# CX9898/BSMR-SDDMM

Measured on AMD Instinct MI355X. Metric: SDDMM GFLOP/s, higher is better.
Workload: dtype f16

## Files before the change

bsmr-sddmm_amd/csrc/gemm_format.hpp:

```cpp
#pragma once

#include <algorithm>
#include <cstdint>
#include <vector>

#include "bsmr_hip.h"
#include "tile_format.hpp"

namespace bsmr {

constexpr uint32_t kGemmWavesM = 2, kGemmWavesN = 4, kGemmWaves = kGemmWavesM * kGemmWavesN;
__host__ __device__ constexpr uint32_t gemmSlabSlot(uint32_t tp, uint32_t r, uint32_t c) { return tp * 256u + (r & 3u) * 64u + (r >> 2) * 16u + c; }
constexpr uint32_t kGemmPassTiles = 16;
constexpr uint32_t kGemmNoEntry = 0xFFFFFFFFu;
constexpr uint32_t kGemmMaxOffset = 8191u;
constexpr uint32_t kGemmSlabStrips = 8;
constexpr uint32_t kGemmWordSlack = 1024;

struct GemmItem {
    uint32_t group;
    uint32_t firstBlock;
    uint32_t listBase;
    uint32_t pad;
};

__host__ __device__ inline void gemmItemPlace(uint32_t i, uint32_t G, uint32_t S, uint32_t& group, uint32_t& strip) {
    const uint32_t slabs = (S + kGemmSlabStrips - 1u) / kGemmSlabStrips;
    uint32_t slab = i / (kGemmSlabStrips * G);
    if (slab >= slabs) slab = slabs - 1u;
    const uint32_t width = slab + 1u < slabs ? kGemmSlabStrips : S - kGemmSlabStrips * (slabs - 1u);
    const uint32_t rem = i - slab * kGemmSlabStrips * G;
    group = rem / width;
    strip = slab * kGemmSlabStrips + rem % width;
}

struct GemmFormatHost {
    uint32_t PM = 0, NB = 0, numGroups = 0, numStrips = 0, passes = 0;
    bool fullGrid = false;
    std::vector<uint32_t> panelRows;
    std::vector<uint32_t> colOf;
    std::vector<GemmItem> items;
    std::vector<uint32_t> rowStart;
    std::vector<uint32_t> lists;
    std::vector<uint32_t> words;
    uint64_t numTiles = 0;
    uint32_t maxListWords = 0;
    size_t bytes() const {
        return 4 * (panelRows.size() + colOf.size() + rowStart.size() + lists.size() + words.size()) + sizeof(GemmItem) * items.size();
    }
};

inline bool gemmShapeOk(uint32_t PM, uint32_t NB) {
    return (PM == 8 || PM == 16) && (NB == 8 || NB == 12 || NB == 16 || NB == 20);
}

inline int packGemm(const HostDense& hd, uint32_t PM, uint32_t NB, GemmFormatHost& out, bool balanceColumns = true) {
    if (!gemmShapeOk(PM, NB)) return BSMR_ERR_INVALID_ARG;
    const uint32_t P = hd.numPanels, TM = PM * 16;
    const uint32_t G = (P + PM - 1) / PM, NCB = (hd.N + 15) / 16, S = (NCB + NB - 1) / NB;
    const uint32_t m = PM / kGemmWavesM, n = NB / kGemmWavesN, Q = (m * n + kGemmPassTiles - 1) / kGemmPassTiles, L = kGemmWaves * Q;
    out = GemmFormatHost();
    out.PM = PM; out.NB = NB; out.numGroups = G; out.numStrips = S; out.passes = Q;
    if (P == 0 || NCB == 0 || hd.entries() == 0) return BSMR_OK;
    if ((uint64_t)G * S > 0x3FFFFFFFull || hd.entries() > 0xFFFFFFF0ull) return BSMR_ERR_INVALID_ARG;
    if ((uint64_t)hd.nnz * 4u > 0xFFFFFFFCull) return BSMR_ERR_INVALID_ARG;
    out.panelRows.assign((size_t)G * TM, hd.panelRows.empty() ? 0u : hd.panelRows[0]);
    std::vector<uint32_t> rowPos((size_t)P * 16);
    if (balanceColumns) {
        std::vector<uint32_t> weight((size_t)P * 16, 0), order((size_t)P * 16);
        for (uint32_t p = 0; p < P; ++p)
            for (uint64_t e = hd.offsets[p]; e < hd.offsets[p + 1]; ++e) ++weight[(size_t)p * 16 + hd.row[e]];
        for (uint32_t i = 0; i < P * 16; ++i) order[i] = i;
        std::stable_sort(order.begin(), order.end(), [&](uint32_t a, uint32_t b) { return weight[a] > weight[b]; });
        const uint32_t bins = 2 * G, half = TM / 2;
        for (uint32_t rank = 0; rank < P * 16; ++rank) {
            const uint32_t round = rank / bins, pos = rank % bins, bin = (round & 1u) ? bins - 1u - pos : pos;
            rowPos[order[rank]] = (bin / 2) * TM + (bin % 2) * half + round;
        }
    } else {
        for (uint32_t i = 0; i < P * 16; ++i) rowPos[i] = i;
    }
    for (uint32_t i = 0; i < P * 16; ++i) out.panelRows[rowPos[i]] = hd.panelRows[i];
    const uint32_t TN = NB * 16;
    std::vector<uint32_t> slotOf(hd.N);
    out.colOf.assign((size_t)S * TN, 0u);
    if (balanceColumns) {
        std::vector<uint32_t> degree(hd.N, 0), hot;
        for (uint64_t e = 0; e < hd.entries(); ++e) ++degree[hd.col[e]];
        uint64_t fullest = 0;
        for (uint32_t st = 0; st < S; ++st) {
            uint64_t sum = 0;
            for (uint32_t c = st * TN; c < std::min<uint64_t>(hd.N, (uint64_t)(st + 1) * TN); ++c) sum += degree[c];
            fullest = std::max(fullest, sum);
        }
        const bool lopsided = fullest * S > 2ull * hd.entries();
        const uint64_t threshold = lopsided ? 2ull * hd.entries() / std::max<uint32_t>(1u, hd.N) + 1ull : ~0ull;
        for (uint32_t c = 0; c < hd.N; ++c)
            if (degree[c] > threshold) hot.push_back(c);
        std::stable_sort(hot.begin(), hot.end(), [&](uint32_t a, uint32_t b) { return degree[a] > degree[b]; });
        std::vector<uint32_t> filled(S, 0);
        for (uint32_t rank = 0; rank < hot.size(); ++rank) {
            const uint32_t round = rank / S, pos = rank % S, strip = (round & 1u) ? S - 1u - pos : pos;
            slotOf[hot[rank]] = strip * TN + filled[strip]++;
        }
        uint32_t strip = 0;
        for (uint32_t c = 0; c < hd.N; ++c) {
            if (degree[c] > threshold) continue;
            while (filled[strip] == TN) ++strip;
            slotOf[c] = strip * TN + filled[strip]++;
        }
    } else {
        for (uint32_t c = 0; c < hd.N; ++c) slotOf[c] = c;
    }
    for (uint32_t c = 0; c < hd.N; ++c) out.colOf[slotOf[c]] = c;
    std::vector<uint32_t> itemOf((size_t)G * S, 0xFFFFFFFFu);
    std::vector<uint8_t> used((size_t)G * S, 0);
    for (uint32_t p = 0; p < P; ++p)
        for (uint64_t e = hd.offsets[p]; e < hd.offsets[p + 1]; ++e)
            used[(size_t)(rowPos[(size_t)p * 16 + hd.row[e]] / TM) * S + slotOf[hd.col[e]] / TN] = 1;
    for (uint32_t i = 0; i < G * S; ++i) {
        uint32_t g, st;
        gemmItemPlace(i, G, S, g, st);
        if (!used[(size_t)g * S + st]) continue;
        itemOf[(size_t)g * S + st] = (uint32_t)out.items.size();
        GemmItem it;
        it.group = g;
        it.firstBlock = st * NB;
        it.listBase = (uint32_t)(out.items.size() * (L + 1));
        it.pad = 0;
        out.items.push_back(it);
    }
    out.fullGrid = out.items.size() == (size_t)G * S;
    const size_t I = out.items.size();
    out.numTiles = (uint64_t)I * PM * NB;
    if (I * (size_t)(L + 1) > 0xFFFFFFFFull || I * (size_t)TM > 0xFFFFFFFFull) return BSMR_ERR_INVALID_ARG;
    out.lists.assign(I * (L + 1), 0);
    out.rowStart.assign(I * TM, 0xFFFFFFFFu);
    auto locate = [&](uint32_t p, uint64_t e, size_t& item, uint32_t& list, uint32_t& slot, uint32_t& rowInWave, uint32_t& rowInTile) {
        const uint32_t place = rowPos[(size_t)p * 16 + hd.row[e]];
        const uint32_t g = place / TM, pj = (place % TM) / 16u;
        const uint32_t slotCol = slotOf[hd.col[e]];
        const uint32_t cb = slotCol >> 4, s = cb / NB, bj = cb % NB;
        const uint32_t wm = pj / m, tm = pj % m, wn = bj / n, tn = bj % n;
        const uint32_t t = tm * n + tn, q = t / kGemmPassTiles, tp = t % kGemmPassTiles;
        const uint32_t r = place & 15u, c = slotCol & 15u;
        item = itemOf[(size_t)g * S + s];
        list = (wm * kGemmWavesN + wn) * Q + q;
        slot = gemmSlabSlot(tp, r, c);
        rowInWave = tm * 16 + r;
        rowInTile = pj * 16 + r;
    };
    for (uint32_t p = 0; p < P; ++p)
        for (uint64_t e = hd.offsets[p]; e < hd.offsets[p + 1]; ++e) {
            size_t item; uint32_t list, slot, rw, rt;
            locate(p, e, item, list, slot, rw, rt);
            ++out.lists[item * (L + 1) + list + 1];
            uint32_t& rs = out.rowStart[item * TM + rt];
            rs = std::min(rs, hd.idx[e]);
        }
    for (uint32_t& v : out.rowStart)
        if (v == 0xFFFFFFFFu) v = 0;
    uint64_t at = 0;
    for (size_t item = 0; item < I; ++item) {
        uint32_t* ls = &out.lists[item * (L + 1)];
        uint64_t run = at;
        for (uint32_t l = 0; l <= L; ++l) {
            const uint32_t cnt = ls[l];
            out.maxListWords = std::max(out.maxListWords, (cnt + 3u) & ~3u);
            run += (cnt + 3u) & ~3u;
            if (run > 0xFFFFFFF0ull) return BSMR_ERR_INVALID_ARG;
            ls[l] = (uint32_t)run;
        }
        at = run;
    }
    if (at > 0xFFFFFFF0ull) return BSMR_ERR_INVALID_ARG;
    out.words.assign((size_t)at + kGemmWordSlack, kGemmNoEntry);
    std::vector<uint32_t> fill(out.lists.size());
    for (size_t item = 0; item < I; ++item)
        for (uint32_t l = 0; l < L; ++l) fill[item * (L + 1) + l] = out.lists[item * (L + 1) + l];
    std::vector<uint64_t> keys(hd.entries());
    for (uint32_t p = 0; p < P; ++p)
        for (uint64_t e = hd.offsets[p]; e < hd.offsets[p + 1]; ++e) {
            size_t item; uint32_t list, slot, rw, rt;
            locate(p, e, item, list, slot, rw, rt);
            const uint32_t off = hd.idx[e] - out.rowStart[item * TM + rt];
            if (off >= kGemmMaxOffset) return BSMR_ERR_BAD_PLAN;
            const uint32_t word = slot | (rw << 12) | (off << 19);
            uint32_t& pos = fill[item * (L + 1) + list];
            keys[e] = ((uint64_t)rw << 45) | ((uint64_t)off << 32) | word;
            out.words[pos++] = (uint32_t)e;
        }
    std::vector<uint64_t> scratch;
    for (size_t item = 0; item < I; ++item)
        for (uint32_t l = 0; l < L; ++l) {
            const uint32_t b = out.lists[item * (L + 1) + l], e = fill[item * (L + 1) + l];
            scratch.resize(e - b);
            for (uint32_t i = b; i < e; ++i) scratch[i - b] = keys[out.words[i]];
            std::sort(scratch.begin(), scratch.end());
            for (uint32_t i = b; i < e; ++i) out.words[i] = (uint32_t)scratch[i - b];
        }
    return BSMR_OK;
}

}
```

bsmr-sddmm_amd/csrc/gemm_kernels.hpp:

```cpp
#pragma once

#include <hip/hip_runtime.h>
#include <stdint.h>

#include "gemm_format.hpp"
#include "sddmm_kernels.hpp"

namespace bsmr {

constexpr uint32_t kGemmBK = 64;
constexpr uint32_t kGemmRowBytes = kGemmBK * 2u;
__host__ __device__ constexpr uint32_t gemmSwz16(uint32_t row) { return (row >> 1) & 7u; }
__host__ __device__ constexpr uint32_t gemmSwz32(uint32_t row) { return ((row >> 1) & 1u) | (((row >> 3) & 1u) * 6u); }
constexpr uint32_t gemmStageBytes(int PM, int NB) { return (uint32_t)(PM + NB) * 16u * kGemmRowBytes; }
constexpr uint32_t kGemmSlabBytes = kGemmPassTiles * 1024u;
constexpr uint32_t gemmRingBytes(int PM, int NB) {
    return 2u * gemmStageBytes(PM, NB) > kGemmWaves * kGemmSlabBytes ? 2u * gemmStageBytes(PM, NB) : kGemmWaves * kGemmSlabBytes;
}
constexpr size_t gemmLdsBytes(int PM, int NB) { return gemmRingBytes(PM, NB) + (size_t)PM * 16u * 4u; }

#if defined(BSMR_GEMM_LAB)
#define GEMM_LAB_ARG , uint32_t labSkip, unsigned long long* labStamps
#define GEMM_LAB_SKIP(bit) (labSkip & (1u << (bit)))
#define GEMM_LAB_STAMPS unsigned long long labStamp[8] = {0, 0, 0, 0, 0, 0, 0, 0}
#define GEMM_LAB_STAMP(i) labStamp[i] = __builtin_amdgcn_s_memrealtime()
#define GEMM_LAB_STAMPS_OUT                                                                              \
    if (labStamps && lane == 0)                                                                          \
        for (uint32_t i = 0; i < 8u; ++i) labStamps[((size_t)blockIdx.x * kGemmWaves + wave) * 8u + i] = labStamp[i]
#else
#define GEMM_LAB_ARG
#define GEMM_LAB_SKIP(bit) false
#define GEMM_LAB_STAMPS
#define GEMM_LAB_STAMP(i)
#define GEMM_LAB_STAMPS_OUT
#endif

__device__ __forceinline__ void gemmKeep(const u32x4& x) {
#if defined(__HIP_DEVICE_COMPILE__)
    asm volatile("" ::"v"(x));
#else
    (void)x;
#endif
}

constexpr uint32_t kGemmDumpHigh = 64764u;
__device__ __forceinline__ void gemmDumpTile(const f32x4& a, uint32_t tileAddr, bool high) {
#if defined(__HIP_DEVICE_COMPILE__)
#pragma clang diagnostic push
#pragma clang diagnostic ignored "-Winline-asm"
    if (!high)
        asm volatile("s_mov_b32 m0, %4\n\ts_nop 0\n\tds_write_addtid_b32 %0\n\tds_write_addtid_b32 %1 offset:256\n\t"
                     "ds_write_addtid_b32 %2 offset:512\n\tds_write_addtid_b32 %3 offset:768"
                     ::"v"(a[0]), "v"(a[1]), "v"(a[2]), "v"(a[3]), "s"(tileAddr) : "memory", "m0");
    else
        asm volatile("s_mov_b32 m0, %4\n\ts_nop 0\n\tds_write_addtid_b32 %0 offset:64764\n\tds_write_addtid_b32 %1 offset:65020\n\t"
                     "ds_write_addtid_b32 %2 offset:65276\n\tds_write_addtid_b32 %3 offset:65532"
                     ::"v"(a[0]), "v"(a[1]), "v"(a[2]), "v"(a[3]), "s"(tileAddr - kGemmDumpHigh) : "memory", "m0");
#pragma clang diagnostic pop
#else
    (void)a; (void)tileAddr; (void)high;
#endif
}
__device__ __forceinline__ uint32_t gemmLdsAddress(const void* p) {
    return (uint32_t)(uintptr_t)(__attribute__((address_space(3))) const void*)p;
}

template <uint32_t DMAS>
__device__ __forceinline__ void gemmStagePart(const uint8_t* src, uint32_t srcBytes, uint8_t* dst, uint32_t wave, const uint32_t* voff, uint32_t kOff) {
    const auto rsrc = __builtin_amdgcn_make_buffer_rsrc(const_cast<uint8_t*>(src), 0, srcBytes, 0x00020000);
#pragma unroll
    for (uint32_t j = 0; j < DMAS; ++j)
        __builtin_amdgcn_raw_ptr_buffer_load_lds(rsrc, (__attribute__((address_space(3))) void*)(dst + (wave * DMAS + j) * 1024u), 16, voff[j], kOff, 0, 0);
}
#if !defined(BSMR_GEMM_BRANCHY_STORES)
__device__ __forceinline__ void gemmStoreEntry(float* P, bool live, uint32_t index, float val) {
    const auto rsrc = __builtin_amdgcn_make_buffer_rsrc(P, 0, 0xFFFFFFFC, 0x00020000);
    __builtin_amdgcn_raw_buffer_store_b32(__builtin_bit_cast(uint32_t, val), rsrc, live ? index << 2 : 0xFFFFFFFFu, 0, 0);
}
#endif
template <uint32_t ADMAS, uint32_t BDMAS>
__device__ __forceinline__ void gemmStage(const uint8_t* A, uint32_t aBytes, const uint8_t* B, uint32_t bBytes, uint8_t* stage, uint32_t bAt,
                                          uint32_t wave, const uint32_t* voffA, const uint32_t* voffB, uint32_t kOff) {
    gemmStagePart<BDMAS>(B, bBytes, stage + bAt, wave, voffB, kOff);
    gemmStagePart<ADMAS>(A, aBytes, stage, wave, voffA, kOff);
}
__device__ __forceinline__ uint32_t gemmRowOfLane(const uint32_t* __restrict__ rows8, uint32_t sub) {
    uint32_t id = rows8[0];
#pragma unroll
    for (uint32_t k = 1; k < 8; ++k) id = sub == k ? rows8[k] : id;
    return id;
}

template <int KT, int PM, int NB, int MODE, bool SRC32 = false>
__global__ void __launch_bounds__(kGemmWaves * kWave, 2)
denseGemm(const void* __restrict__ Aop, const void* __restrict__ Bop, uint32_t aBytes, uint32_t bBytes,
          const uint32_t* __restrict__ panelRows, const uint32_t* __restrict__ colOf, const GemmItem* __restrict__ items,
          const uint32_t* __restrict__ rowStart,
          const uint32_t* __restrict__ lists, const uint32_t* __restrict__ words, float* __restrict__ P, uint32_t N,
          uint32_t gridG, uint32_t gridS, uint32_t fullGrid, Batch batch GEMM_LAB_ARG) {
    constexpr uint32_t ESZ = SRC32 ? 4u : 2u, K = (kGemmRowBytes / ESZ) * KT, TM = PM * 16u, TN = NB * 16u;
    constexpr uint32_t KSUB = SRC32 ? 1u : 2u;
    constexpr uint32_t m = PM / kGemmWavesM, n = NB / kGemmWavesN, Q = (m * n + kGemmPassTiles - 1u) / kGemmPassTiles, L = kGemmWaves * Q;
    constexpr uint32_t ADMAS = PM / 4u, BDMAS = NB / 4u;
    static_assert(PM % 4 == 0 && NB % 4 == 0, "a stage is filled in whole 1-KiB pieces per wave");
    constexpr uint32_t stageBytes = gemmStageBytes(PM, NB), bAt = TM * kGemmRowBytes;
    constexpr uint32_t rowTableAt = gemmRingBytes(PM, NB);
    constexpr uint32_t kGemmWordChunk = m * n > 32u ? 4u : 8u;
    constexpr bool kPlainDump = m * n > 32u;

    extern __shared__ __attribute__((aligned(16))) uint8_t lds[];
    const uint32_t itemId = xcdContiguous(blockIdx.x, gridDim.x);
    uint32_t group, firstBlock, listBase;
    if (fullGrid) {
        gemmItemPlace(itemId, gridG, gridS, group, firstBlock);
        firstBlock *= (uint32_t)NB;
        listBase = itemId * (L + 1u);
    } else {
        const GemmItem item = items[itemId];
        group = item.group;
        firstBlock = item.firstBlock;
        listBase = item.listBase;
    }
    const uint32_t wave = __builtin_amdgcn_readfirstlane(threadIdx.x >> 6), lane = threadIdx.x & 63u;
    const uint32_t wm = wave / kGemmWavesN, wn = wave % kGemmWavesN;
    const uint32_t r = lane & 15u, g = lane >> 4;
    GEMM_LAB_STAMPS;
    GEMM_LAB_STAMP(0);

    const uint8_t* Ab = static_cast<const uint8_t*>(Aop) + (size_t)blockIdx.y * batch.strideA * ESZ;
    const uint8_t* Bb = static_cast<const uint8_t*>(Bop) + (size_t)blockIdx.y * batch.strideB * ESZ;
    P += (size_t)blockIdx.y * batch.strideP;

    uint32_t voffA[ADMAS], voffB[BDMAS];
#pragma unroll
    for (uint32_t j = 0; j < BDMAS; ++j) {
        const uint32_t col = 8u * (wave * BDMAS + j) + (lane >> 3);
        const uint32_t id = gemmRowOfLane(colOf + (size_t)firstBlock * 16u + 8u * (wave * BDMAS + j), lane >> 3);
        voffB[j] = id * (K * ESZ) + (((lane & 7u) ^ (SRC32 ? gemmSwz32(col) : gemmSwz16(col))) << 4);
    }
    if (!GEMM_LAB_SKIP(2)) gemmStagePart<BDMAS>(Bb, bBytes, lds + bAt, wave, voffB, 0u);
#pragma unroll
    for (uint32_t j = 0; j < ADMAS; ++j) {
        const uint32_t row = 8u * (wave * ADMAS + j) + (lane >> 3);
        const uint32_t id = gemmRowOfLane(panelRows + (size_t)group * TM + 8u * (wave * ADMAS + j), lane >> 3);
        voffA[j] = id * (K * ESZ) + (((lane & 7u) ^ (SRC32 ? gemmSwz32(row) : gemmSwz16(row))) << 4);
    }
    if (!GEMM_LAB_SKIP(2)) gemmStagePart<ADMAS>(Ab, aBytes, lds, wave, voffA, 0u);
    GEMM_LAB_STAMP(1);
    if (threadIdx.x < TM) reinterpret_cast<uint32_t*>(lds + rowTableAt)[threadIdx.x] = rowStart[(size_t)itemId * TM + threadIdx.x];
    uint32_t myList[Q + 1];
#pragma unroll
    for (uint32_t q = 0; q <= Q; ++q) myList[q] = lists[listBase + wave * Q + q];

    const uint32_t fragOff = r * kGemmRowBytes + ((SRC32 ? (2u * g) ^ gemmSwz32(r) : g ^ gemmSwz16(r)) << 4);
    const uint32_t aRead = wm * (TM / 2u) * kGemmRowBytes + fragOff;
    const uint32_t bRead = bAt + wn * (TN / 4u) * kGemmRowBytes + fragOff;

    f32x4 acc[m][n];
#pragma unroll
    for (uint32_t i = 0; i < m; ++i)
#pragma unroll
        for (uint32_t j = 0; j < n; ++j) acc[i][j] = f32x4{0.f, 0.f, 0.f, 0.f};

    auto loadWords = [&](uint32_t e0, uint32_t (&w)[kGemmWordChunk]) {
#pragma unroll
        for (uint32_t u = 0; u < kGemmWordChunk; ++u) w[u] = GEMM_LAB_SKIP(4) ? kGemmNoEntry : words[e0 + u * kWave + lane];
    };
    constexpr bool kDeepWords = Q >= 2u && m * n <= 32u;
    uint32_t wAhead[2][kGemmWordChunk];

    asm volatile("s_waitcnt vmcnt(0)" ::: "memory");
    GEMM_LAB_STAMP(2);
    __builtin_amdgcn_s_barrier();
    GEMM_LAB_STAMP(3);
    constexpr bool kEarlyWords = KT <= 4;
    if (kEarlyWords) {
        loadWords(myList[0], wAhead[0]);
        if (kDeepWords) loadWords(myList[1], wAhead[1]);
    }

#pragma unroll
    for (uint32_t t = 0; t < (uint32_t)KT; ++t) {
        if (t + 1u < (uint32_t)KT && !GEMM_LAB_SKIP(2))
            gemmStage<ADMAS, BDMAS>(Ab, aBytes, Bb, bBytes, lds + ((t + 1u) & 1u) * stageBytes, bAt, wave, voffA, voffB, (t + 1u) * kGemmRowBytes);
        if (!kEarlyWords && t + 1u == (uint32_t)KT) {
            loadWords(myList[0], wAhead[0]);
            if (kDeepWords) loadWords(myList[1], wAhead[1]);
        }
        const uint8_t* base = lds + (t & 1u) * stageBytes;
#pragma unroll
        for (uint32_t s = 0; s < KSUB; ++s) {
            auto fragment = [&](uint32_t at, uint32_t tile, uint32_t tag) -> u32x4 {
                if (GEMM_LAB_SKIP(1)) return u32x4{lane, t, tile, s + tag};
                const uint8_t* src = base + ((at + tile * 16u * kGemmRowBytes) ^ (s << 6));
                if constexpr (SRC32) {
                    const f32x4 lo = *reinterpret_cast<const f32x4*>(src);
                    const f32x4 hi = *reinterpret_cast<const f32x4*>(reinterpret_cast<const uint8_t*>(reinterpret_cast<uintptr_t>(src) ^ 16u));
                    return packLowp<MODE>(lo, hi);
                } else {
                    return *reinterpret_cast<const u32x4*>(src);
                }
            };
            u32x4 bf[n];
#pragma unroll
            for (uint32_t j = 0; j < n; ++j) bf[j] = fragment(bRead, j, 0u);
#pragma unroll
            for (uint32_t i = 0; i < m; ++i) {
                const u32x4 af = fragment(aRead, i, 2u);
                if (!GEMM_LAB_SKIP(0)) {
#pragma unroll
                    for (uint32_t j = 0; j < n; ++j) acc[i][j] = mfma16<MODE>(af, bf[j], acc[i][j]);
                } else {
                    gemmKeep(af);
#pragma unroll
                    for (uint32_t j = 0; j < n; ++j) gemmKeep(bf[j]);
                }
            }
        }
        asm volatile("s_waitcnt vmcnt(0) lgkmcnt(0)" ::: "memory");
        __builtin_amdgcn_s_barrier();
    }

    GEMM_LAB_STAMP(4);
    float* slab = reinterpret_cast<float*>(lds) + wave * (kGemmPassTiles * 256u);
    const uint32_t slabAddr = __builtin_amdgcn_readfirstlane(gemmLdsAddress(slab));
    const uint32_t* rowTable = reinterpret_cast<const uint32_t*>(lds + rowTableAt) + wm * (TM / 2u);
#pragma unroll
    for (uint32_t q = 0; q < Q; ++q) {
        if (!GEMM_LAB_SKIP(3)) {
            if (kPlainDump) {
#pragma unroll
                for (uint32_t tp = 0; tp < kGemmPassTiles; ++tp) {
                    const uint32_t tIdx = q * kGemmPassTiles + tp;
                    if (tIdx < m * n) {
#pragma unroll
                        for (uint32_t j = 0; j < 4u; ++j) slab[tp * 256u + j * 64u + lane] = acc[tIdx / n][tIdx % n][j];
                    }
                }
            } else if (slabAddr < 0x10000u) {
#pragma unroll
                for (uint32_t tp = 0; tp < kGemmPassTiles; ++tp) {
                    const uint32_t tIdx = q * kGemmPassTiles + tp;
                    if (tIdx < m * n) gemmDumpTile(acc[tIdx / n][tIdx % n], slabAddr + tp * 1024u, false);
                }
            } else {
#pragma unroll
                for (uint32_t tp = 0; tp < kGemmPassTiles; ++tp) {
                    const uint32_t tIdx = q * kGemmPassTiles + tp;
                    if (tIdx < m * n) gemmDumpTile(acc[tIdx / n][tIdx % n], slabAddr + tp * 1024u, true);
                }
            }
        }
        const uint32_t first = myList[q], last = myList[q + 1u];
        uint32_t w[kGemmWordChunk];
#pragma unroll
        for (uint32_t u = 0; u < kGemmWordChunk; ++u) w[u] = wAhead[q & 1u][u];
        if (kDeepWords) {
            if (q + 2u < Q) loadWords(myList[q + 2u], wAhead[q & 1u]);
        } else if (q + 1u < Q) {
            loadWords(last, wAhead[(q + 1u) & 1u]);
        }
        for (uint32_t e = first; e < last; e += kGemmWordChunk * kWave) {
            if (e != first) loadWords(e, w);
#pragma unroll
            for (uint32_t u = 0; u < kGemmWordChunk; ++u) {
#if defined(BSMR_GEMM_BRANCHY_STORES)
                if (e + u * kWave + lane < last && w[u] != kGemmNoEntry) {
                    const float val = slab[w[u] & 4095u];
                    const uint32_t dst = rowTable[(w[u] >> 12) & 127u] + (w[u] >> 19);
                    if (!GEMM_LAB_SKIP(5)) P[dst] = val;
                }
#else
                const bool live = e + u * kWave + lane < last && w[u] != kGemmNoEntry;
                const float val = slab[w[u] & 4095u];
                const uint32_t dst = rowTable[(w[u] >> 12) & (TM / 2u - 1u)] + (w[u] >> 19);
                if (!GEMM_LAB_SKIP(5)) gemmStoreEntry(P, live, dst, val);
#endif
            }
        }
        GEMM_LAB_STAMP(5u + q);
    }
    GEMM_LAB_STAMPS_OUT;
}

constexpr uint32_t kGemmHalfRowBytes = 64u;
__host__ __device__ constexpr uint32_t gemmSwzH(uint32_t row) { return (4u - ((row >> 2) & 3u)) & 3u; }
constexpr uint32_t gemmCvtRingBytes(int PM, int NB) {
    const uint32_t used = (uint32_t)(PM + NB) * 16u * (kGemmRowBytes + 2u * kGemmHalfRowBytes);
    return used > kGemmWaves * kGemmSlabBytes ? used : kGemmWaves * kGemmSlabBytes;
}
constexpr size_t gemmCvtLdsBytes(int PM, int NB) { return gemmCvtRingBytes(PM, NB) + (size_t)PM * 16u * 4u; }

template <int KT, int PM, int NB, int MODE>
__global__ void __launch_bounds__(kGemmWaves * kWave, 2)
denseGemmCvt(const float* __restrict__ Aop, const float* __restrict__ Bop, uint32_t aBytes, uint32_t bBytes,
             const uint32_t* __restrict__ panelRows, const uint32_t* __restrict__ colOf, const GemmItem* __restrict__ items,
             const uint32_t* __restrict__ rowStart,
             const uint32_t* __restrict__ lists, const uint32_t* __restrict__ words, float* __restrict__ P, uint32_t N,
             uint32_t gridG, uint32_t gridS, uint32_t fullGrid, Batch batch GEMM_LAB_ARG) {
    constexpr uint32_t K = 32u * KT, TM = PM * 16u, TN = NB * 16u, ROWS = TM + TN;
    constexpr uint32_t m = PM / kGemmWavesM, n = NB / kGemmWavesN, Q = (m * n + kGemmPassTiles - 1u) / kGemmPassTiles, L = kGemmWaves * Q;
    constexpr uint32_t ADMAS = PM / 4u, BDMAS = NB / 4u, DMAS = ADMAS + BDMAS;
    constexpr uint32_t fBytes = ROWS * kGemmRowBytes, hBytes = ROWS * kGemmHalfRowBytes, bAtF = TM * kGemmRowBytes, bAtH = TM * kGemmHalfRowBytes;
    constexpr uint32_t hAt = fBytes, rowTableAt = gemmCvtRingBytes(PM, NB);
    constexpr uint32_t kGemmWordChunk = m * n > 32u ? 4u : 8u;

    extern __shared__ __attribute__((aligned(16))) uint8_t lds[];
    const uint32_t itemId = xcdContiguous(blockIdx.x, gridDim.x);
    uint32_t group, firstBlock, listBase;
    if (fullGrid) {
        gemmItemPlace(itemId, gridG, gridS, group, firstBlock);
        firstBlock *= (uint32_t)NB;
        listBase = itemId * (L + 1u);
    } else {
        const GemmItem item = items[itemId];
        group = item.group;
        firstBlock = item.firstBlock;
        listBase = item.listBase;
    }
    const uint32_t wave = __builtin_amdgcn_readfirstlane(threadIdx.x >> 6), lane = threadIdx.x & 63u;
    const uint32_t wm = wave / kGemmWavesN, wn = wave % kGemmWavesN;
    const uint32_t r = lane & 15u, g = lane >> 4;
    GEMM_LAB_STAMPS;
    GEMM_LAB_STAMP(0);
    const uint8_t* Ab = reinterpret_cast<const uint8_t*>(Aop) + (size_t)blockIdx.y * batch.strideA * 4u;
    const uint8_t* Bb = reinterpret_cast<const uint8_t*>(Bop) + (size_t)blockIdx.y * batch.strideB * 4u;
    P += (size_t)blockIdx.y * batch.strideP;

    uint32_t voffA[ADMAS], voffB[BDMAS];
    const uint32_t piece = lane & 7u;
#pragma unroll
    for (uint32_t j = 0; j < BDMAS; ++j)
        voffB[j] = gemmRowOfLane(colOf + (size_t)firstBlock * 16u + 8u * (wave * BDMAS + j), lane >> 3) * (K * 4u) + (piece << 4);
    if (!GEMM_LAB_SKIP(2)) gemmStagePart<BDMAS>(Bb, bBytes, lds + bAtF, wave, voffB, 0u);
#pragma unroll
    for (uint32_t j = 0; j < ADMAS; ++j)
        voffA[j] = gemmRowOfLane(panelRows + (size_t)group * TM + 8u * (wave * ADMAS + j), lane >> 3) * (K * 4u) + (piece << 4);
    if (!GEMM_LAB_SKIP(2)) gemmStagePart<ADMAS>(Ab, aBytes, lds, wave, voffA, 0u);
    GEMM_LAB_STAMP(1);
    if (threadIdx.x < TM) reinterpret_cast<uint32_t*>(lds + rowTableAt)[threadIdx.x] = rowStart[(size_t)itemId * TM + threadIdx.x];
    uint32_t myList[Q + 1];
#pragma unroll
    for (uint32_t q = 0; q <= Q; ++q) myList[q] = lists[listBase + wave * Q + q];

#if defined(BSMR_GEMM_ROUND_SERIAL)
    constexpr uint32_t kRoundBatch = 1u;
#else
    constexpr uint32_t kRoundBatch = 5u;
#endif
    const uint32_t fOfA = wave * ADMAS * 1024u + lane * 16u, fOfB = bAtF + wave * BDMAS * 1024u + lane * 16u;
    auto hOf = [&](uint32_t part, uint32_t firstChunk, uint32_t odd) {
        const uint32_t quarter = (2u * (firstChunk + odd) + (lane >> 5)) & 3u;
        return hAt + part + firstChunk * 512u + (lane >> 3) * kGemmHalfRowBytes + (((piece >> 1) ^ ((4u - quarter) & 3u)) << 4) + ((piece & 1u) << 3);
    };
    const uint32_t hOfA[2] = {hOf(0u, wave * ADMAS, 0u), hOf(0u, wave * ADMAS, 1u)};
    const uint32_t hOfB[2] = {hOf(bAtH, wave * BDMAS, 0u), hOf(bAtH, wave * BDMAS, 1u)};
    auto roundChunks = [&](uint32_t to) {
        if (GEMM_LAB_SKIP(1)) return;
#pragma unroll
        for (uint32_t j0 = 0; j0 < DMAS; j0 += kRoundBatch) {
            f32x4 v[kRoundBatch];
#pragma unroll
            for (uint32_t b = 0; b < kRoundBatch; ++b) {
                const uint32_t j = j0 + b;
                if (j >= DMAS) continue;
                v[b] = j < ADMAS ? *reinterpret_cast<const f32x4*>(lds + fOfA + j * 1024u)
                                 : *reinterpret_cast<const f32x4*>(lds + fOfB + (j - ADMAS) * 1024u);
            }
#pragma unroll
            for (uint32_t b = 0; b < kRoundBatch; ++b) {
                const uint32_t j = j0 + b;
                if (j >= DMAS) continue;
                const uint32_t jj = j < ADMAS ? j : j - ADMAS;
                uint8_t* dst = lds + (j < ADMAS ? hOfA[jj & 1u] : hOfB[jj & 1u]) + jj * 512u + to * hBytes;
                typedef uint32_t u32x2 __attribute__((ext_vector_type(2)));
                u32x2 h;
                if constexpr (MODE == 0) {
                    typedef _Float16 f16x4 __attribute__((ext_vector_type(4)));
                    f16x4 o;
                    o[0] = (_Float16)v[b][0]; o[1] = (_Float16)v[b][1]; o[2] = (_Float16)v[b][2]; o[3] = (_Float16)v[b][3];
                    h = __builtin_bit_cast(u32x2, o);
                } else {
                    typedef __bf16 bf16x4 __attribute__((ext_vector_type(4)));
                    bf16x4 o;
                    o[0] = (__bf16)v[b][0]; o[1] = (__bf16)v[b][1]; o[2] = (__bf16)v[b][2]; o[3] = (__bf16)v[b][3];
                    h = __builtin_bit_cast(u32x2, o);
                }
                *reinterpret_cast<u32x2*>(dst) = h;
            }
        }
    };

    const uint32_t fragOff = r * kGemmHalfRowBytes + ((g ^ gemmSwzH(r)) << 4);
    const uint32_t aRead = wm * (TM / 2u) * kGemmHalfRowBytes + fragOff;
    const uint32_t bRead = bAtH + wn * (TN / 4u) * kGemmHalfRowBytes + fragOff;

    f32x4 acc[m][n];
#pragma unroll
    for (uint32_t i = 0; i < m; ++i)
#pragma unroll
        for (uint32_t j = 0; j < n; ++j) acc[i][j] = f32x4{0.f, 0.f, 0.f, 0.f};
    auto loadWords = [&](uint32_t e0, uint32_t (&w)[kGemmWordChunk]) {
#pragma unroll
        for (uint32_t u = 0; u < kGemmWordChunk; ++u) w[u] = GEMM_LAB_SKIP(4) ? kGemmNoEntry : words[e0 + u * kWave + lane];
    };
    constexpr bool kDeepWords = Q >= 2u && m * n <= 32u;
    uint32_t wAhead[2][kGemmWordChunk];

    asm volatile("s_waitcnt vmcnt(0)" ::: "memory");
    GEMM_LAB_STAMP(2);
    roundChunks(0u);
    asm volatile("s_waitcnt lgkmcnt(0)" ::: "memory");
    if (KT > 1 && !GEMM_LAB_SKIP(2)) gemmStage<ADMAS, BDMAS>(Ab, aBytes, Bb, bBytes, lds, bAtF, wave, voffA, voffB, kGemmRowBytes);
    __builtin_amdgcn_s_barrier();
    GEMM_LAB_STAMP(3);
    constexpr bool kEarlyWords = KT <= 4;
    if (kEarlyWords) {
        loadWords(myList[0], wAhead[0]);
        if (kDeepWords) loadWords(myList[1], wAhead[1]);
    }

#pragma unroll
    for (uint32_t t = 0; t < (uint32_t)KT; ++t) {
        if (!kEarlyWords && t + 1u == (uint32_t)KT) {
            loadWords(myList[0], wAhead[0]);
            if (kDeepWords) loadWords(myList[1], wAhead[1]);
        }
        const uint8_t* base = lds + hAt + (t & 1u) * hBytes;
        u32x4 bf[n];
#pragma unroll
        for (uint32_t j = 0; j < n; ++j)
            bf[j] = GEMM_LAB_SKIP(6) ? u32x4{lane, t, j, 0u} : *reinterpret_cast<const u32x4*>(base + bRead + j * 16u * kGemmHalfRowBytes);
#pragma unroll
        for (uint32_t i = 0; i < m; ++i) {
            const u32x4 af = GEMM_LAB_SKIP(6) ? u32x4{lane, t, i, 2u} : *reinterpret_cast<const u32x4*>(base + aRead + i * 16u * kGemmHalfRowBytes);
            if (!GEMM_LAB_SKIP(0)) {
#pragma unroll
                for (uint32_t j = 0; j < n; ++j) acc[i][j] = mfma16<MODE>(af, bf[j], acc[i][j]);
            } else {
                gemmKeep(af);
#pragma unroll
                for (uint32_t j = 0; j < n; ++j) gemmKeep(bf[j]);
            }
        }
        if (t + 1u < (uint32_t)KT) {
            asm volatile("s_waitcnt vmcnt(0)" ::: "memory");
            roundChunks((t + 1u) & 1u);
            asm volatile("s_waitcnt lgkmcnt(0)" ::: "memory");
            if (t + 2u < (uint32_t)KT && !GEMM_LAB_SKIP(2))
                gemmStage<ADMAS, BDMAS>(Ab, aBytes, Bb, bBytes, lds, bAtF, wave, voffA, voffB, (t + 2u) * kGemmRowBytes);
        } else {
            asm volatile("s_waitcnt lgkmcnt(0)" ::: "memory");
        }
        __builtin_amdgcn_s_barrier();
    }

    GEMM_LAB_STAMP(4);
    float* slab = reinterpret_cast<float*>(lds) + wave * (kGemmPassTiles * 256u);
    const uint32_t slabAddr = __builtin_amdgcn_readfirstlane(gemmLdsAddress(slab));
    const uint32_t* rowTable = reinterpret_cast<const uint32_t*>(lds + rowTableAt) + wm * (TM / 2u);
#pragma unroll
    for (uint32_t q = 0; q < Q; ++q) {
        if (!GEMM_LAB_SKIP(3)) {
            if (slabAddr < 0x10000u) {
#pragma unroll
                for (uint32_t tp = 0; tp < kGemmPassTiles; ++tp) {
                    const uint32_t tIdx = q * kGemmPassTiles + tp;
                    if (tIdx < m * n) gemmDumpTile(acc[tIdx / n][tIdx % n], slabAddr + tp * 1024u, false);
                }
            } else {
#pragma unroll
                for (uint32_t tp = 0; tp < kGemmPassTiles; ++tp) {
                    const uint32_t tIdx = q * kGemmPassTiles + tp;
                    if (tIdx < m * n) gemmDumpTile(acc[tIdx / n][tIdx % n], slabAddr + tp * 1024u, true);
                }
            }
        }
        const uint32_t first = myList[q], last = myList[q + 1u];
        uint32_t w[kGemmWordChunk];
#pragma unroll
        for (uint32_t u = 0; u < kGemmWordChunk; ++u) w[u] = wAhead[q & 1u][u];
        if (kDeepWords) {
            if (q + 2u < Q) loadWords(myList[q + 2u], wAhead[q & 1u]);
        } else if (q + 1u < Q) {
            loadWords(last, wAhead[(q + 1u) & 1u]);
        }
        for (uint32_t e = first; e < last; e += kGemmWordChunk * kWave) {
            if (e != first) loadWords(e, w);
#pragma unroll
            for (uint32_t u = 0; u < kGemmWordChunk; ++u) {
#if defined(BSMR_GEMM_BRANCHY_STORES)
                if (e + u * kWave + lane < last && w[u] != kGemmNoEntry) {
                    const float val = slab[w[u] & 4095u];
                    const uint32_t dst = rowTable[(w[u] >> 12) & 127u] + (w[u] >> 19);
                    if (!GEMM_LAB_SKIP(5)) P[dst] = val;
                }
#else
                const bool live = e + u * kWave + lane < last && w[u] != kGemmNoEntry;
                const float val = slab[w[u] & 4095u];
                const uint32_t dst = rowTable[(w[u] >> 12) & (TM / 2u - 1u)] + (w[u] >> 19);
                if (!GEMM_LAB_SKIP(5)) gemmStoreEntry(P, live, dst, val);
#endif
            }
        }
        GEMM_LAB_STAMP(5u + q);
    }
    GEMM_LAB_STAMPS_OUT;
}

}
```

Baseline: 15390.

## Prefetch mask words ahead, balance rows across passes, load words before barrier

The scatter loop over mask words now software-pipelines the word loads, fetching the next chunk while the current chunk's stores are issued instead of loading at the top of each iteration. The first word loads move ahead of the waitcnt/barrier by default so their latency overlaps the staging wait. On the host, row placement during column balancing now picks the row tile within each bin that keeps per-pass store load most even. The goal is to hide global load latency in the epilogue and even out epilogue work across passes, at the cost of more live registers and more host-side preprocessing.

```diff
diff --git a/bsmr-sddmm_amd/csrc/gemm_format.hpp b/bsmr-sddmm_amd/csrc/gemm_format.hpp
--- a/bsmr-sddmm_amd/csrc/gemm_format.hpp
+++ b/bsmr-sddmm_amd/csrc/gemm_format.hpp
@@ -16,6 +16,7 @@
 constexpr uint32_t kGemmMaxOffset = 8191u;
 constexpr uint32_t kGemmSlabStrips = 8;
 constexpr uint32_t kGemmWordSlack = 1024;
+constexpr uint32_t kGemmMaxRowTiles = 8, kGemmMaxPasses = 3;
 
 struct GemmItem {
     uint32_t group;
@@ -73,9 +74,25 @@
         for (uint32_t i = 0; i < P * 16; ++i) order[i] = i;
         std::stable_sort(order.begin(), order.end(), [&](uint32_t a, uint32_t b) { return weight[a] > weight[b]; });
         const uint32_t bins = 2 * G, half = TM / 2;
+        uint32_t share[kGemmMaxRowTiles][kGemmMaxPasses] = {};
+        for (uint32_t tm = 0; tm < m; ++tm)
+            for (uint32_t tn = 0; tn < n; ++tn) ++share[tm][(tm * n + tn) / kGemmPassTiles];
+        std::vector<uint64_t> load((size_t)bins * Q, 0);
+        std::vector<uint8_t> rowsIn((size_t)bins * m, 0);
         for (uint32_t rank = 0; rank < P * 16; ++rank) {
             const uint32_t round = rank / bins, pos = rank % bins, bin = (round & 1u) ? bins - 1u - pos : pos;
-            rowPos[order[rank]] = (bin / 2) * TM + (bin % 2) * half + round;
+            const uint64_t w = weight[order[rank]];
+            uint64_t* ld = &load[(size_t)bin * Q];
+            uint32_t best = m;
+            uint64_t bestFullest = 0;
+            for (uint32_t tm = 0; tm < m; ++tm) {
+                if (rowsIn[(size_t)bin * m + tm] == 16) continue;
+                uint64_t fullest = 0;
+                for (uint32_t q = 0; q < Q; ++q) fullest = std::max(fullest, ld[q] + w * share[tm][q]);
+                if (best == m || fullest < bestFullest) { best = tm; bestFullest = fullest; }
+            }
+            for (uint32_t q = 0; q < Q; ++q) ld[q] += w * share[best][q];
+            rowPos[order[rank]] = (bin / 2) * TM + (bin % 2) * half + best * 16u + rowsIn[(size_t)bin * m + best]++;
         }
     } else {
         for (uint32_t i = 0; i < P * 16; ++i) rowPos[i] = i;
diff --git a/bsmr-sddmm_amd/csrc/gemm_kernels.hpp b/bsmr-sddmm_amd/csrc/gemm_kernels.hpp
--- a/bsmr-sddmm_amd/csrc/gemm_kernels.hpp
+++ b/bsmr-sddmm_amd/csrc/gemm_kernels.hpp
@@ -72,12 +72,55 @@
     for (uint32_t j = 0; j < DMAS; ++j)
         __builtin_amdgcn_raw_ptr_buffer_load_lds(rsrc, (__attribute__((address_space(3))) void*)(dst + (wave * DMAS + j) * 1024u), 16, voff[j], kOff, 0, 0);
 }
-#if !defined(BSMR_GEMM_BRANCHY_STORES)
 __device__ __forceinline__ void gemmStoreEntry(float* P, bool live, uint32_t index, float val) {
     const auto rsrc = __builtin_amdgcn_make_buffer_rsrc(P, 0, 0xFFFFFFFC, 0x00020000);
     __builtin_amdgcn_raw_buffer_store_b32(__builtin_bit_cast(uint32_t, val), rsrc, live ? index << 2 : 0xFFFFFFFFu, 0, 0);
 }
-#endif
+template <uint32_t C>
+__device__ __forceinline__ void gemmLoadWords(const uint32_t* __restrict__ words, uint32_t e0, uint32_t lane, uint32_t (&w)[C], bool skip) {
+    const uint32_t* __restrict__ base = words + e0;
+#pragma unroll
+    for (uint32_t u = 0; u < C; ++u) w[u] = skip ? kGemmNoEntry : base[u * kWave + lane];
+}
+template <uint32_t C, uint32_t HALF>
+__device__ __forceinline__ void gemmMaskTrip(const float* slab, const uint32_t* rowTable, float* P, uint32_t e, uint32_t last, uint32_t lane,
+                                             const uint32_t (&w)[C], bool skipStores) {
+#pragma unroll
+    for (uint32_t u = 0; u < C; ++u) {
+        const bool live = e + u * kWave + lane < last && w[u] != kGemmNoEntry;
+        const float val = slab[w[u] & 4095u];
+        const uint32_t dst = rowTable[(w[u] >> 12) & (HALF - 1u)] + (w[u] >> 19);
+        if (!skipStores) gemmStoreEntry(P, live, dst, val);
+    }
+}
+template <uint32_t C, uint32_t HALF, uint32_t Q, bool DEEP>
+__device__ __forceinline__ void gemmMaskPass(const uint32_t* __restrict__ words, const float* slab, const uint32_t* rowTable, float* P,
+                                             const uint32_t (&myList)[Q + 1u], uint32_t q, uint32_t lane, uint32_t (&wAhead)[2][C],
+                                             bool skipLoads, bool skipStores) {
+    const uint32_t first = myList[q], last = myList[q + 1u];
+    uint32_t w[C];
+#pragma unroll
+    for (uint32_t u = 0; u < C; ++u) w[u] = wAhead[q & 1u][u];
+    if (DEEP) {
+        if (q + 2u < Q) gemmLoadWords<C>(words, myList[q + 2u], lane, wAhead[q & 1u], skipLoads);
+    } else if (q + 1u < Q) {
+        gemmLoadWords<C>(words, last, lane, wAhead[(q + 1u) & 1u], skipLoads);
+    }
+    constexpr uint32_t T = C * kWave;
+    const bool more = first + T < last;
+    uint32_t over[C];
+    if (more) gemmLoadWords<C>(words, first + T, lane, over, skipLoads);
+    gemmMaskTrip<C, HALF>(slab, rowTable, P, first, last, lane, w, skipStores);
+    if (more) {
+        for (uint32_t e = first + T; e < last; e += T) {
+            uint32_t ahead[C];
+            gemmLoadWords<C>(words, e + T, lane, ahead, skipLoads);
+            gemmMaskTrip<C, HALF>(slab, rowTable, P, e, last, lane, over, skipStores);
+#pragma unroll
+            for (uint32_t u = 0; u < C; ++u) over[u] = ahead[u];
+        }
+    }
+}
 template <uint32_t ADMAS, uint32_t BDMAS>
 __device__ __forceinline__ void gemmStage(const uint8_t* A, uint32_t aBytes, const uint8_t* B, uint32_t bBytes, uint8_t* stage, uint32_t bAt,
                                           uint32_t wave, const uint32_t* voffA, const uint32_t* voffB, uint32_t kOff) {
@@ -162,31 +205,31 @@
 #pragma unroll
         for (uint32_t j = 0; j < n; ++j) acc[i][j] = f32x4{0.f, 0.f, 0.f, 0.f};
 
-    auto loadWords = [&](uint32_t e0, uint32_t (&w)[kGemmWordChunk]) {
-#pragma unroll
-        for (uint32_t u = 0; u < kGemmWordChunk; ++u) w[u] = GEMM_LAB_SKIP(4) ? kGemmNoEntry : words[e0 + u * kWave + lane];
-    };
+    auto loadWords = [&](uint32_t e0, uint32_t (&w)[kGemmWordChunk]) { gemmLoadWords<kGemmWordChunk>(words, e0, lane, w, GEMM_LAB_SKIP(4)); };
     constexpr bool kDeepWords = Q >= 2u && m * n <= 32u;
     uint32_t wAhead[2][kGemmWordChunk];
+    constexpr bool kEarlyWords = KT <= 4 && !kPlainDump;
+    auto firstWords = [&]() {
+        loadWords(myList[0], wAhead[0]);
+        if (kDeepWords) loadWords(myList[1], wAhead[1]);
+    };
+#if !defined(BSMR_GEMM_LATE_WORDS)
+    if (kEarlyWords) firstWords();
+#endif
 
     asm volatile("s_waitcnt vmcnt(0)" ::: "memory");
     GEMM_LAB_STAMP(2);
     __builtin_amdgcn_s_barrier();
     GEMM_LAB_STAMP(3);
-    constexpr bool kEarlyWords = KT <= 4;
-    if (kEarlyWords) {
-        loadWords(myList[0], wAhead[0]);
-        if (kDeepWords) loadWords(myList[1], wAhead[1]);
-    }
+#if defined(BSMR_GEMM_LATE_WORDS)
+    if (kEarlyWords) firstWords();
+#endif
 
 #pragma unroll
     for (uint32_t t = 0; t < (uint32_t)KT; ++t) {
         if (t + 1u < (uint32_t)KT && !GEMM_LAB_SKIP(2))
             gemmStage<ADMAS, BDMAS>(Ab, aBytes, Bb, bBytes, lds + ((t + 1u) & 1u) * stageBytes, bAt, wave, voffA, voffB, (t + 1u) * kGemmRowBytes);
-        if (!kEarlyWords && t + 1u == (uint32_t)KT) {
-            loadWords(myList[0], wAhead[0]);
-            if (kDeepWords) loadWords(myList[1], wAhead[1]);
-        }
+        if (!kEarlyWords && t + 1u == (uint32_t)KT) firstWords();
         const uint8_t* base = lds + (t & 1u) * stageBytes;
 #pragma unroll
         for (uint32_t s = 0; s < KSUB; ++s) {
@@ -251,33 +294,8 @@
                 }
             }
         }
-        const uint32_t first = myList[q], last = myList[q + 1u];
-        uint32_t w[kGemmWordChunk];
-#pragma unroll
-        for (uint32_t u = 0; u < kGemmWordChunk; ++u) w[u] = wAhead[q & 1u][u];
-        if (kDeepWords) {
-            if (q + 2u < Q) loadWords(myList[q + 2u], wAhead[q & 1u]);
-        } else if (q + 1u < Q) {
-            loadWords(last, wAhead[(q + 1u) & 1u]);
-        }
-        for (uint32_t e = first; e < last; e += kGemmWordChunk * kWave) {
-            if (e != first) loadWords(e, w);
-#pragma unroll
-            for (uint32_t u = 0; u < kGemmWordChunk; ++u) {
-#if defined(BSMR_GEMM_BRANCHY_STORES)
-                if (e + u * kWave + lane < last && w[u] != kGemmNoEntry) {
-                    const float val = slab[w[u] & 4095u];
-                    const uint32_t dst = rowTable[(w[u] >> 12) & 127u] + (w[u] >> 19);
-                    if (!GEMM_LAB_SKIP(5)) P[dst] = val;
-                }
-#else
-                const bool live = e + u * kWave + lane < last && w[u] != kGemmNoEntry;
-                const float val = slab[w[u] & 4095u];
-                const uint32_t dst = rowTable[(w[u] >> 12) & (TM / 2u - 1u)] + (w[u] >> 19);
-                if (!GEMM_LAB_SKIP(5)) gemmStoreEntry(P, live, dst, val);
-#endif
-            }
-        }
+        if (kPlainDump) __builtin_amdgcn_sched_barrier(0);
+        gemmMaskPass<kGemmWordChunk, TM / 2u, Q, kDeepWords>(words, slab, rowTable, P, myList, q, lane, wAhead, GEMM_LAB_SKIP(4), GEMM_LAB_SKIP(5));
         GEMM_LAB_STAMP(5u + q);
     }
     GEMM_LAB_STAMPS_OUT;
@@ -400,12 +418,17 @@
     for (uint32_t i = 0; i < m; ++i)
 #pragma unroll
         for (uint32_t j = 0; j < n; ++j) acc[i][j] = f32x4{0.f, 0.f, 0.f, 0.f};
-    auto loadWords = [&](uint32_t e0, uint32_t (&w)[kGemmWordChunk]) {
-#pragma unroll
-        for (uint32_t u = 0; u < kGemmWordChunk; ++u) w[u] = GEMM_LAB_SKIP(4) ? kGemmNoEntry : words[e0 + u * kWave + lane];
-    };
+    auto loadWords = [&](uint32_t e0, uint32_t (&w)[kGemmWordChunk]) { gemmLoadWords<kGemmWordChunk>(words, e0, lane, w, GEMM_LAB_SKIP(4)); };
     constexpr bool kDeepWords = Q >= 2u && m * n <= 32u;
     uint32_t wAhead[2][kGemmWordChunk];
+    constexpr bool kEarlyWords = KT <= 4;
+    auto firstWords = [&]() {
+        loadWords(myList[0], wAhead[0]);
+        if (kDeepWords) loadWords(myList[1], wAhead[1]);
+    };
+#if !defined(BSMR_GEMM_LATE_WORDS)
+    if (kEarlyWords) firstWords();
+#endif
 
     asm volatile("s_waitcnt vmcnt(0)" ::: "memory");
     GEMM_LAB_STAMP(2);
@@ -414,18 +437,13 @@
     if (KT > 1 && !GEMM_LAB_SKIP(2)) gemmStage<ADMAS, BDMAS>(Ab, aBytes, Bb, bBytes, lds, bAtF, wave, voffA, voffB, kGemmRowBytes);
     __builtin_amdgcn_s_barrier();
     GEMM_LAB_STAMP(3);
-    constexpr bool kEarlyWords = KT <= 4;
-    if (kEarlyWords) {
-        loadWords(myList[0], wAhead[0]);
-        if (kDeepWords) loadWords(myList[1], wAhead[1]);
-    }
+#if defined(BSMR_GEMM_LATE_WORDS)
+    if (kEarlyWords) firstWords();
+#endif
 
 #pragma unroll
     for (uint32_t t = 0; t < (uint32_t)KT; ++t) {
-        if (!kEarlyWords && t + 1u == (uint32_t)KT) {
-            loadWords(myList[0], wAhead[0]);
-            if (kDeepWords) loadWords(myList[1], wAhead[1]);
-        }
+        if (!kEarlyWords && t + 1u == (uint32_t)KT) firstWords();
         const uint8_t* base = lds + hAt + (t & 1u) * hBytes;
         u32x4 bf[n];
 #pragma unroll
@@ -476,33 +494,7 @@
                 }
             }
         }
-        const uint32_t first = myList[q], last = myList[q + 1u];
-        uint32_t w[kGemmWordChunk];
-#pragma unroll
-        for (uint32_t u = 0; u < kGemmWordChunk; ++u) w[u] = wAhead[q & 1u][u];
-        if (kDeepWords) {
-            if (q + 2u < Q) loadWords(myList[q + 2u], wAhead[q & 1u]);
-        } else if (q + 1u < Q) {
-            loadWords(last, wAhead[(q + 1u) & 1u]);
-        }
-        for (uint32_t e = first; e < last; e += kGemmWordChunk * kWave) {
-            if (e != first) loadWords(e, w);
-#pragma unroll
-            for (uint32_t u = 0; u < kGemmWordChunk; ++u) {
-#if defined(BSMR_GEMM_BRANCHY_STORES)
-                if (e + u * kWave + lane < last && w[u] != kGemmNoEntry) {
-                    const float val = slab[w[u] & 4095u];
-                    const uint32_t dst = rowTable[(w[u] >> 12) & 127u] + (w[u] >> 19);
-                    if (!GEMM_LAB_SKIP(5)) P[dst] = val;
-                }
-#else
-                const bool live = e + u * kWave + lane < last && w[u] != kGemmNoEntry;
-                const float val = slab[w[u] & 4095u];
-                const uint32_t dst = rowTable[(w[u] >> 12) & (TM / 2u - 1u)] + (w[u] >> 19);
-                if (!GEMM_LAB_SKIP(5)) gemmStoreEntry(P, live, dst, val);
-#endif
-            }
-        }
+        gemmMaskPass<kGemmWordChunk, TM / 2u, Q, kDeepWords>(words, slab, rowTable, P, myList, q, lane, wAhead, GEMM_LAB_SKIP(4), GEMM_LAB_SKIP(5));
         GEMM_LAB_STAMP(5u + q);
     }
     GEMM_LAB_STAMPS_OUT;
```

Result: faster. 16160 (median of 6 runs) (+5.0%).
